# zhengjingsen/LidarDetection

Measured on AMD Instinct MI355X. Metric: frames/sec (fwd+NMS) PointPillar-KITTI, higher is better.
Workload: dtype f32; 1 GPU; PointPillar-KITTI bs=16 per GPU, fp32, eval BN folded: HIP voxelize + PFN; dense 2D backbone = first layer from the pillars (sparse implicit GEMM), stride-1 3x3 layers as Winograd F(4x4,3x3) on the fp32 MFMA, strided deblocks as one fused MFMA GEMM (all this repo's HIP), the two stride-2 3x3 layers MIOpen, stride-1 deblock + 1x1 heads hipBLASLt; exact HIP top-k + decode + batched rotated NMS; clou; replicas=1

## Files before the change

include/lidar_hip.h:

```cpp
#ifndef LIDAR_HIP_H
#define LIDAR_HIP_H

#include <stddef.h>
#include <stdint.h>

#ifdef __cplusplus
extern "C" {
#endif

#define LIDAR_OK 0
#define LIDAR_ERR_ARG (-1)
#define LIDAR_ERR_LAUNCH (-2)
#define LIDAR_ERR_WORKSPACE (-3)
#define LIDAR_ERR_UNSUPPORTED (-4)

size_t lidar_voxelize_workspace_bytes(int batch, int n_max, int max_voxels);
int lidar_voxelize_workspace_init(void *ws, size_t ws_bytes, int batch, int n_max, int max_voxels, void *stream);
int lidar_voxelize(const float *points, const int *point_offsets, int batch, int n_max, int num_features,
                   const float *range6, const float *voxel_size3, const int *grid3, int max_points,
                   int max_voxels, int compact, int algo, float *voxels, int *coords, int *num_points,
                   int *voxel_offsets, void *ws, size_t ws_bytes, void *stream);
int lidar_voxelize_hostoff(const float *points, const int *point_offsets, const int *host_offsets, int batch, int n_max,
                           int num_features, const float *range6, const float *voxel_size3, const int *grid3, int max_points,
                           int max_voxels, int compact, int algo, float *voxels, int *coords, int *num_points,
// ... 155 lines not shown
                               const float *weight, const float *bias, float *out_features, void *stream);
int lidar_spconv_implicit_gemm_fused(const float *in_features, const int *nbr, int n_out, int K, int Cin, int Cout,
                                     const float *weight, const float *bias, const float *residual, int relu,
                                     float *out_features, void *stream);
int lidar_spconv_row_masks(const int *nbr, int n_out, int K, int *masks, void *stream);
size_t lidar_spconv_mask_group_workspace_bytes(int n_out);
int lidar_spconv_mask_group_init(void *ws, size_t ws_bytes, void *stream);
int lidar_spconv_mask_group(const int *nbr, int n_out, int K, int *masks, int *order, void *ws, size_t ws_bytes, void *stream);
int lidar_spconv_sorted_gemm_supported(int K, int Cin, int Cout);
int lidar_spconv_implicit_gemm_sorted(const float *in_features, const int *nbr, const int *row_mask, const int *order,
                                      int n_out, int K, int Cin, int Cout, const float *weight, const float *bias,
                                      const float *residual, int relu, float *out_features, void *stream);
size_t lidar_spconv_packed_floats(int K, int Cin, int Cout);
int lidar_spconv_pack_weights(const float *weight, int K, int Cin, int Cout, float *packed, void *stream);
int lidar_spconv_implicit_gemm_sorted_packed(const float *in_features, const int *nbr, const int *row_mask, const int *order,
                                             int n_out, int K, int Cin, int Cout, const float *packed, const float *bias,
                                             const float *residual, int relu, float *out_features, void *stream);
int lidar_spconv_wgrad(const float *in_features, const float *grad_out, const int *nbr, int n_out, int K, int Cin, int Cout,
                       float *grad_weight, void *stream);
int lidar_spconv_wgrad_mfma_supported(int K, int Cin, int Cout);
size_t lidar_spconv_wgrad_workspace_bytes(int n_out, int K, int Cin, int Cout);
int lidar_spconv_wgrad_mfma(const float *in_features, const float *grad_out, const int *nbr, const int *order, int n_out, int K,
                            int Cin, int Cout, float *grad_weight, void *ws, size_t ws_bytes, void *stream);
size_t lidar_sparse_to_dense_workspace_bytes(int batch, int D, int H, int W);
int lidar_sparse_to_dense(const float *features, const int *indices, int n, int channels, int batch, int D, int H, int W,
                          float *out, void *ws, size_t ws_bytes, void *stream);

int lidar_bias_act_nhwc(const float *in, const float *bias, long long n_pix, int C, int relu, float *out, int out_C,
                        int out_off, void *stream);
int lidar_bias_act_upsample_nhwc(const float *in, const float *bias, int batch, int h, int w, int s, int C, int relu,
                                 float *out, int out_C, int out_off, void *stream);
int lidar_dense_gemm_bias_act(const float *A, long long M, int K, const float *W, int N, const float *bias, int relu,
                              float *D, int ldd, void *ws, size_t ws_bytes, void *stream);
int lidar_dense_gemm_export_choices(int *out7, int cap);
int lidar_dense_gemm_import_choices(const int *in7, int n);

size_t lidar_wino_packed_floats(int Cin, int Cout);
int lidar_wino_supported(int Cin, int Cout);
int lidar_wino_pack_weights(const float *w, int Cin, int Cout, float *packed, void *stream);
int lidar_wino_conv3x3_nhwc(const float *in, int B, int H, int W, int Cin, const float *packed, const float *bias, int relu, int Cout,
                            float *out, int out_C, int out_off, void *stream);
int lidar_wino_conv3x3_grouped_nhwc(const float *in, int B, int H, int W, int in_C, int group_cin, int n_groups, const float *packed,
                                    const float *bias, int relu, float *out, int out_C, int out_off, void *stream);
int lidar_wino_conv3x3_grouped_compact_nhwc(const float *in, int B, int H, int W, int in_C, int group_cin, int n_groups,
                                            const float *packed, const float *bias, int relu, const int *grp_cout, const int *grp_ooff,
                                            float *out, int out_C, int out_off, void *stream);

size_t lidar_wino43_packed_floats(int Cin, int Cout);
int lidar_wino43_supported(int Cin, int Cout);
int lidar_wino43_pack_weights(const float *w, int Cin, int Cout, float *packed, void *stream);
int lidar_wino43_conv3x3_nhwc(const float *in, int B, int H, int W, int Cin, int in_C, const float *packed, const float *bias, int relu,
                              int Cout, float *out, int out_C, int out_off, void *stream);

int lidar_wino43_wgrad_supported(int Cin, int Cout);
size_t lidar_wino43_wgrad_workspace_bytes(int B, int H, int W, int Cin, int Cout);
int lidar_wino43_wgrad_nhwc(const float *x, int x_ld, const float *g, int g_ld, int B, int H, int W, int Cin, int Cout, float *dw,
                            void *ws, size_t ws_bytes, void *stream);

size_t lidar_deconv_packed_floats(int K, int N);
int lidar_deconv_supported(int K, int s, int C_up);
int lidar_deconv_pack_weights(const float *W, int K, int N, float *packed, void *stream);
int lidar_deconv_gemm_nhwc(const float *in, int B, int h, int w, int K, const float *packed, const float *bias, int relu, int s, int C_up,
                           float *out, int out_C, int out_off, void *stream);

#define LIDAR_DECONV_TRAIN_MIN_K 16
#define LIDAR_DECONV_TRAIN_MIN_CUP 32
#define LIDAR_DECONV_TRAIN_MAX_C 512
int lidar_deconv_train_supported(int K, int s, int C_up);
size_t lidar_deconv_wgrad_workspace_bytes(int B, int h, int w, int K, int s, int C_up);
int lidar_deconv_dgrad_nhwc(const float *g, int g_ld, const float *W, int B, int h, int w, int K, int s, int C_up, float *dx, int dx_ld,
                            void *stream);
int lidar_deconv_wgrad_nhwc(const float *x, int x_ld, const float *g, int g_ld, int B, int h, int w, int K, int s, int C_up, float *dw,
                            void *ws, size_t ws_bytes, void *stream);

int lidar_anchor_scores(const float *head, long long n_loc, int row_stride, int cls_off, int anchors_per_loc, int num_class,
                        float score_thresh, float *scores, unsigned char *labels, void *stream);
int lidar_decode_topk(const float *head, int batch, long long locs_per_frame, int row_stride, int box_off, int dir_off,
                      int anchors_per_loc, int num_dir_bins, const long long *top_idx, int k, const float *anchors,
                      float dir_offset, float dir_limit_offset, float period, float *boxes, void *stream);
size_t lidar_topk_workspace_bytes(int batch, long long n);
int lidar_topk_workspace_init(void *ws, size_t ws_bytes, int batch, long long n, void *stream);
int lidar_anchor_scores_hist(const float *head, int batch, long long locs_per_frame, int row_stride, int cls_off, int anchors_per_loc,
                             int num_class, float score_thresh, float *scores, unsigned char *labels, void *ws, size_t ws_bytes,
                             void *stream);
int lidar_topk_desc(const float *scores, int batch, long long n, int k, float valid_min, float score_max, int hist_ready,
                    float *top_scores, long long *top_idx, int *counts, void *ws, size_t ws_bytes, void *stream);
int lidar_post_nms_gather(const float *boxes, const float *top_scores, const long long *top_idx, const unsigned char *labels,
                          const long long *keep, const int *num_keep, int batch, int k, long long n, int keep_stride, int post,
                          float *out_boxes, float *out_scores, long long *out_labels, int *out_num, void *stream);

size_t lidar_anchor_assign_workspace_bytes(int batch, int max_gt, int num_classes);
int lidar_anchor_assign(const float *const *anchors, const long long *counts, const long long *per_loc, const long long *out_off,
                        const float *matched, const float *unmatched, const int *remap, int num_classes, int anchor_dim,
                        long long a_total, const signed char *class_of_id, const float *gt, const float *gt_enlarged, int batch,
                        int max_gt, int gt_cols, int code_size, int sincos, int norm_by_num_examples, int *labels, float *targets,
                        float *weights, void *ws, size_t ws_bytes, void *stream);

size_t lidar_anchor_loss_workspace_bytes(int batch, const long long *counts, int num_heads);
int lidar_anchor_loss_forward(const float *const *cls, const float *const *box, const float *const *dir, const long long *counts,
                              const int *cols, const int *col_off, int num_heads, const int *labels, const float *targets,
                              const float *anchors, int anchor_dim, int batch, long long n_total, int num_class, int code_size,
                              int num_dir_bins, const float *code_weights, const float *weights, int flags, float *losses, void *ws,
                              size_t ws_bytes, void *stream);
int lidar_anchor_loss_backward(const float *const *cls, const float *const *box, const float *const *dir, const long long *counts,
                               const int *cols, const int *col_off, int num_heads, const int *labels, const float *targets,
                               const float *anchors, int anchor_dim, int batch, long long n_total, int num_class, int code_size,
// ... 17 lines not shown
```

lidardetection_amd/_lib.py:

```python
import ctypes as C
import os

_HERE = os.path.dirname(os.path.abspath(__file__))
SO_PATH = os.environ.get("LIDAR_HIP_SO") or os.path.join(_HERE, "csrc", "liblidar_hip.so")

vp, i32, f32, sz = C.c_void_p, C.c_int, C.c_float, C.c_size_t

SIGNATURES = {
    "lidar_voxelize_workspace_bytes": (sz, [i32, i32, i32]),
    "lidar_voxelize_workspace_init": (i32, [vp, sz, i32, i32, i32, vp]),
    "lidar_voxelize": (i32, [vp, vp, i32, i32, i32, vp, vp, vp, i32, i32, i32, i32, vp, vp, vp, vp, vp, sz, vp]),
    "lidar_voxelize_hostoff": (i32, [vp, vp, vp, i32, i32, i32, vp, vp, vp, i32, i32, i32, i32, vp, vp, vp, vp, vp, sz, vp]),
    "lidar_voxelize_error_flag": (i32, [vp, sz, i32, i32, i32]),
    "lidar_timer_create": (vp, []),
    "lidar_timer_destroy": (None, [vp]),
    "lidar_voxelize_time_next": (None, [vp]),
    "lidar_timer_elapsed_ms": (C.c_float, [vp]),
    "lidar_timer_parts_ms": (i32, [vp, vp]),
    "lidar_voxelize_set_error_mirror": (i32, [vp, sz, i32, i32, i32, vp, vp]),
    "lidar_pillar_vfe": (i32, [vp, vp, vp, i32, vp, i32, i32, vp, vp, vp, i32, vp, vp, i32, i32, i32, vp, vp]),
    "lidar_mean_vfe": (i32, [vp, vp, i32, i32, i32, i32, vp, vp]),
    "lidar_pillar_scatter_workspace_bytes": (sz, [i32, i32, i32]),
    "lidar_pillar_scatter": (i32, [vp, vp, i32, i32, vp, i32, i32, i32, i32, i32, vp, vp, sz, vp]),
    "lidar_pillar_scatter_update": (i32, [vp, vp, i32, i32, vp, i32, i32, i32, i32, vp, vp, vp, vp]),
# ... 35 lines not shown
    "lidar_gather_points_grad_batch": (i32, [i32, i32, i32, i32, vp, vp, vp, vp]),
    "lidar_three_nn_batch": (i32, [i32, i32, i32, vp, vp, vp, vp, vp]),
    "lidar_three_interpolate_batch": (i32, [i32, i32, i32, i32, vp, vp, vp, vp, vp]),
    "lidar_three_interpolate_grad_batch": (i32, [i32, i32, i32, i32, vp, vp, vp, vp, vp]),
    "lidar_roiaware_pool3d_forward": (i32, [i32, i32, i32, i32, i32, i32, i32, vp, vp, vp, vp, vp, vp, i32, vp]),
    "lidar_roiaware_pool3d_backward": (i32, [i32, i32, i32, i32, i32, i32, vp, vp, vp, vp, i32, vp]),
    "lidar_points_in_boxes": (i32, [i32, i32, i32, vp, vp, vp, vp]),
    "lidar_roipoint_pool3d_forward": (i32, [i32, i32, i32, i32, i32, vp, vp, vp, vp, vp, vp]),
    "lidar_spconv_hash_capacity": (sz, [i32]),
    "lidar_spconv_build_hash": (i32, [vp, i32, i32, i32, i32, vp, sz, vp]),
    "lidar_spconv_subm_table": (i32, [vp, i32, i32, i32, i32, i32, i32, i32, vp, sz, vp, vp]),
    "lidar_spconv_conv_table_workspace_bytes": (sz, [i32, i32, i32, i32, i32, i32, i32]),
    "lidar_spconv_conv_outputs": (i32, [vp, i32, i32, i32, i32, i32, i32, i32, i32, i32, i32, i32, i32, i32, i32, vp, i32, vp, vp, sz, vp]),
    "lidar_spconv_conv_tables": (i32, [i32, i32, i32, i32, i32, i32, i32, i32, vp, vp, vp, sz, vp]),
    "lidar_spconv_grid_init": (i32, [vp, sz, vp]),
    "lidar_spconv_grid_rows": (i32, [vp, i32, vp, i32, i32, i32, i32, vp, i32, vp]),
    "lidar_spconv_grid_table": (i32, [vp, i32, i32, i32, i32, i32, i32, i32, i32, i32, i32, i32, i32, i32, i32, vp, i32, vp, vp]),
    "lidar_spconv_grid_table_t": (i32, [vp, i32, i32, i32, i32, i32, i32, i32, i32, i32, i32, i32, i32, i32, i32, vp, i32, vp, vp]),
    "lidar_spconv_grid_pad_rows": (i32, [vp, vp, i32, vp]),
    "lidar_spconv_transpose_table": (i32, [vp, i32, i32, i32, vp, vp]),
    "lidar_spconv_grid_outputs_workspace_bytes": (sz, [i32, i32]),
    "lidar_spconv_grid_outputs": (i32, [vp, i32, i32, i32, i32, i32, i32, i32, i32, i32, i32, i32, i32, i32, i32, vp, vp, vp, vp, sz, vp]),
    "lidar_spconv_implicit_gemm": (i32, [vp, vp, i32, i32, i32, i32, vp, vp, vp, vp]),
    "lidar_spconv_implicit_gemm_fused": (i32, [vp, vp, i32, i32, i32, i32, vp, vp, vp, i32, vp, vp]),
    "lidar_spconv_row_masks": (i32, [vp, i32, i32, vp, vp]),
    "lidar_spconv_mask_group_workspace_bytes": (sz, [i32]),
    "lidar_spconv_mask_group_init": (i32, [vp, sz, vp]),
    "lidar_spconv_mask_group": (i32, [vp, i32, i32, vp, vp, vp, sz, vp]),
    "lidar_spconv_sorted_gemm_supported": (i32, [i32, i32, i32]),
    "lidar_spconv_implicit_gemm_sorted": (i32, [vp, vp, vp, vp, i32, i32, i32, i32, vp, vp, vp, i32, vp, vp]),
    "lidar_spconv_packed_floats": (sz, [i32, i32, i32]),
    "lidar_spconv_pack_weights": (i32, [vp, i32, i32, i32, vp, vp]),
    "lidar_spconv_implicit_gemm_sorted_packed": (i32, [vp, vp, vp, vp, i32, i32, i32, i32, vp, vp, vp, i32, vp, vp]),
    "lidar_spconv_wgrad": (i32, [vp, vp, vp, i32, i32, i32, i32, vp, vp]),
    "lidar_spconv_wgrad_mfma_supported": (i32, [i32, i32, i32]),
    "lidar_spconv_wgrad_workspace_bytes": (sz, [i32, i32, i32, i32]),
    "lidar_spconv_wgrad_mfma": (i32, [vp, vp, vp, vp, i32, i32, i32, i32, vp, vp, sz, vp]),
    "lidar_sparse_to_dense_workspace_bytes": (sz, [i32, i32, i32, i32]),
    "lidar_sparse_to_dense": (i32, [vp, vp, i32, i32, i32, i32, i32, i32, vp, vp, sz, vp]),
    "lidar_sparse_to_bev_nhwc": (i32, [vp, vp, i32, i32, i32, i32, i32, i32, vp, vp, sz, vp]),
    "lidar_bias_act_nhwc": (i32, [vp, vp, C.c_longlong, i32, i32, vp, i32, i32, vp]),
    "lidar_bias_act_upsample_nhwc": (i32, [vp, vp, i32, i32, i32, i32, i32, i32, vp, i32, i32, vp]),
    "lidar_dense_gemm_bias_act": (i32, [vp, C.c_longlong, i32, vp, i32, vp, i32, vp, i32, vp, sz, vp]),
    "lidar_dense_gemm_export_choices": (i32, [vp, i32]),
    "lidar_dense_gemm_import_choices": (i32, [vp, i32]),
    "lidar_wino_packed_floats": (sz, [i32, i32]),
    "lidar_wino_supported": (i32, [i32, i32]),
    "lidar_wino_pack_weights": (i32, [vp, i32, i32, vp, vp]),
    "lidar_wino_conv3x3_nhwc": (i32, [vp, i32, i32, i32, i32, vp, vp, i32, i32, vp, i32, i32, vp]),
    "lidar_wino43_packed_floats": (sz, [i32, i32]),
    "lidar_wino43_supported": (i32, [i32, i32]),
    "lidar_wino43_pack_weights": (i32, [vp, i32, i32, vp, vp]),
    "lidar_wino43_conv3x3_nhwc": (i32, [vp, i32, i32, i32, i32, i32, vp, vp, i32, i32, vp, i32, i32, vp]),
    "lidar_wino43_wgrad_supported": (i32, [i32, i32]),
    "lidar_wino43_wgrad_workspace_bytes": (sz, [i32, i32, i32, i32, i32]),
    "lidar_wino43_wgrad_nhwc": (i32, [vp, i32, vp, i32, i32, i32, i32, i32, i32, vp, vp, sz, vp]),
    "lidar_wino_conv3x3_grouped_nhwc": (i32, [vp, i32, i32, i32, i32, i32, i32, vp, vp, i32, vp, i32, i32, vp]),
    "lidar_wino_conv3x3_grouped_compact_nhwc": (i32, [vp, i32, i32, i32, i32, i32, i32, vp, vp, i32, vp, vp, vp, i32, i32, vp]),
    "lidar_deconv_packed_floats": (sz, [i32, i32]),
    "lidar_deconv_supported": (i32, [i32, i32, i32]),
    "lidar_deconv_pack_weights": (i32, [vp, i32, i32, vp, vp]),
    "lidar_deconv_gemm_nhwc": (i32, [vp, i32, i32, i32, i32, vp, vp, i32, i32, i32, vp, i32, i32, vp]),
    "lidar_deconv_train_supported": (i32, [i32, i32, i32]),
    "lidar_deconv_wgrad_workspace_bytes": (sz, [i32, i32, i32, i32, i32, i32]),
    "lidar_deconv_dgrad_nhwc": (i32, [vp, i32, vp, i32, i32, i32, i32, i32, i32, vp, i32, vp]),
    "lidar_deconv_wgrad_nhwc": (i32, [vp, i32, vp, i32, i32, i32, i32, i32, i32, i32, vp, vp, sz, vp]),
    "lidar_anchor_scores": (i32, [vp, C.c_longlong, i32, i32, i32, i32, f32, vp, vp, vp]),
    "lidar_decode_topk": (i32, [vp, i32, C.c_longlong, i32, i32, i32, i32, i32, vp, i32, vp, f32, f32, f32, vp, vp]),
    "lidar_topk_workspace_bytes": (sz, [i32, C.c_longlong]),
    "lidar_topk_workspace_init": (i32, [vp, sz, i32, C.c_longlong, vp]),
    "lidar_anchor_scores_hist": (i32, [vp, i32, C.c_longlong, i32, i32, i32, i32, f32, vp, vp, vp, sz, vp]),
    "lidar_topk_desc": (i32, [vp, i32, C.c_longlong, i32, f32, f32, i32, vp, vp, vp, vp, sz, vp]),
    "lidar_post_nms_gather": (i32, [vp, vp, vp, vp, vp, vp, i32, i32, C.c_longlong, i32, i32, vp, vp, vp, vp, vp]),
    "lidar_anchor_assign_workspace_bytes": (sz, [i32, i32, i32]),
    "lidar_anchor_assign": (i32, [vp, vp, vp, vp, vp, vp, vp, i32, i32, C.c_longlong, vp, vp, vp, i32, i32, i32, i32, i32, i32, vp,
                                  vp, vp, vp, sz, vp]),
    "lidar_anchor_loss_workspace_bytes": (sz, [i32, vp, i32]),
    "lidar_anchor_loss_forward": (i32, [vp, vp, vp, vp, vp, vp, i32, vp, vp, vp, i32, i32, C.c_longlong, i32, i32, i32, vp, vp, i32,
                                        vp, vp, sz, vp]),
    "lidar_anchor_loss_backward": (i32, [vp, vp, vp, vp, vp, vp, i32, vp, vp, vp, i32, i32, C.c_longlong, i32, i32, i32, vp, vp, i32,
                                         vp, vp, vp, vp, vp, sz, vp]),
    "lidar_rotate_iou_eval": (i32, [vp, i32, vp, i32, i32, vp, vp]),
    "lidar_boxes_iou_bev_cpu": (i32, [vp, i32, vp, i32, vp]),
    "lidar_points_in_boxes_cpu": (i32, [vp, i32, vp, i32, vp]),
    "lidar_voxelize_cpu_scratch_bytes": (sz, [i32]),
    "lidar_voxelize_cpu": (i32, [vp, i32, i32, vp, vp, vp, i32, i32, vp, vp, vp, vp, sz]),
}

_lib = None


class LidarHipError(RuntimeError):
    pass


def lib():
    global _lib
    if _lib is None:
        if not os.path.exists(SO_PATH):
            raise LidarHipError(
                f"{SO_PATH} is missing: build it with `python -c 'import __graft_entry__ as g; g.build()'` "
                "(hipcc --offload-arch=gfx950). There is no CPU fallback.")
        _lib = C.CDLL(SO_PATH)
        for name, (res, args) in SIGNATURES.items():
            fn = getattr(_lib, name)
            fn.restype = res
# ... 88 lines not shown
```

lidardetection_amd/bev_backbone.py:

```python
import ctypes as C
import os
from typing import NamedTuple, Optional

import torch
import torch.nn as nn
import torch.nn.functional as F

from . import _lib, wino, workspace


def bias_act_(x, bias, relu=True, out=None, out_offset=0):
    _lib.require_cuda(bias)
    if not (x.is_cuda and x.dim() == 4 and x.is_contiguous(memory_format=torch.channels_last)):
        raise _lib.LidarHipError("bias_act_: expected a channels-last CUDA tensor")
    B, C, H, W = x.shape
    out, out_offset = (x, 0) if out is None else _lib.nhwc_out("bias_act_", B, (H, W), C, x.device, out, out_offset)
    _lib.check(_lib.lib().lidar_bias_act_nhwc(_lib.ptr(x), _lib.ptr(bias), B * H * W, C, int(bool(relu)), _lib.ptr(out),
                                              out.shape[1], int(out_offset), _lib.stream()), "lidar_bias_act_nhwc")
    return out


_LT_GEMM = [os.environ.get("LIDAR_BEV_LT_GEMM", "1") != "0"]
_SPLIT_MIN = [int(os.environ.get("LIDAR_BEV_SPLIT_MIN", "8"))]
_SPLIT = [int(os.environ.get("LIDAR_BEV_SPLIT", "2"))]
_WINO = [os.environ.get("LIDAR_BEV_WINO", "1") != "0"]
_DECONV = [os.environ.get("LIDAR_BEV_DECONV", "1") != "0"]
_SPARSE_FIRST = [os.environ.get("LIDAR_BEV_SPARSE_FIRST", "1") != "0"]


def _lt_gemm(a_ptr, M, K, w_kn, bias, relu, d_ptr, ldd, device):
    ws = workspace.get("dense_gemm", 32 << 20, device)
    st = _lib.lib().lidar_dense_gemm_bias_act(a_ptr, M, K, _lib.ptr(w_kn), w_kn.shape[1], _lib.ptr(bias), int(bool(relu)), d_ptr, ldd,
                                              _lib.ptr(ws), ws.numel(), _lib.stream())
    if st == -4:
        return False
    _lib.check(st, "lidar_dense_gemm_bias_act")
    return True


def _side_streams(device, n):
    from .spconv import conv as _sc, modules as _sm
    dev = torch.device(device)
    out = []
    for pool in (_sc._SIDE_STREAMS, _sm._RULEBOOK_STREAMS)[:n]:
        st = pool.get(dev)
        if st is None:
            st = pool[dev] = torch.cuda.Stream(dev, priority=-1)
        out.append(st)
    return out


def gemm_bias_act_into_(x, w_kn, bias, out, out_offset, relu=True):
    _lib.require_cuda(w_kn, bias)
    _lib.require_nhwc(x, "gemm_bias_act_into_")
    B, K, h, w = x.shape
    N = w_kn.shape[1]
    if w_kn.shape[0] != K or bias.numel() != N:
        raise _lib.LidarHipError("gemm_bias_act_into_: shapes do not match")
    out, out_offset = _lib.nhwc_out("gemm_bias_act_into_", B, (h, w), N, x.device, out, out_offset)
    return _lt_gemm(_lib.ptr(x), B * h * w, K, w_kn, bias, relu, C.c_void_p(out.data_ptr() + 4 * out_offset), out.shape[1], x.device)


def rows_gemm(a2d, w_kn, bias=None, out=None):
    if _LT_GEMM[0] and a2d.is_cuda and a2d.dtype == torch.float32 and a2d.is_contiguous() and w_kn.is_contiguous():
        if out is None:
            out = torch.empty((a2d.shape[0], w_kn.shape[1]), dtype=torch.float32, device=a2d.device)
        elif not out.is_contiguous() or out.shape != (a2d.shape[0], w_kn.shape[1]):
            raise _lib.LidarHipError("rows_gemm: out must be a contiguous (M, N) tensor")
        if _lt_gemm(_lib.ptr(a2d), a2d.shape[0], a2d.shape[1], w_kn, bias, False, _lib.ptr(out), w_kn.shape[1], a2d.device):
            return out
        _LT_GEMM[0] = False
    if out is None:
        return torch.mm(a2d, w_kn) if bias is None else torch.addmm(bias, a2d, w_kn)
    return torch.mm(a2d, w_kn, out=out) if bias is None else torch.addmm(bias, a2d, w_kn, out=out)


def deconv_supported(K, s, c_up):
    return bool(_lib.lib().lidar_deconv_supported(int(K), int(s), int(c_up)))


def deconv_pack(w_kn):
    _lib.require_cuda(w_kn)
    K, N = w_kn.shape
    L = _lib.lib()
    n = L.lidar_deconv_packed_floats(K, N)
    if n == 0:
        raise _lib.LidarHipError(f"deconv_pack: unsupported shape ({K}, {N})")
    packed = torch.empty(n, dtype=torch.float32, device=w_kn.device)
    _lib.check(L.lidar_deconv_pack_weights(_lib.ptr(w_kn.contiguous()), K, N, _lib.ptr(packed), _lib.stream()), "lidar_deconv_pack_weights")
    return packed


_DECONV_MAX_BYTES = [2 ** 31 - 1]


def deconv_fits(B, K, h, w, s, out_c):
    return B * h * w * K * 4 < _DECONV_MAX_BYTES[0] and B * h * w * s * s * out_c * 4 < _DECONV_MAX_BYTES[0]


def deconv_gemm_into_(x, packed, bias, s, out, out_offset=0, relu=True):
    _lib.require_cuda(packed, bias)
    _lib.require_nhwc(x, "deconv_gemm_into_")
    B, K, h, w = x.shape
    c_up = bias.numel()
    if packed.numel() != K * s * s * c_up:
        raise _lib.LidarHipError("deconv_gemm_into_: packed weights do not match (K, s, C_up)")
    out, out_offset = _lib.nhwc_out("deconv_gemm_into_", B, (s * h, s * w), c_up, x.device, out, out_offset)
    _lib.check(_lib.lib().lidar_deconv_gemm_nhwc(_lib.ptr(x), B, h, w, K, _lib.ptr(packed), _lib.ptr(bias), int(bool(relu)), int(s), c_up,
                                                 _lib.ptr(out), out.shape[1], int(out_offset), _lib.stream()), "lidar_deconv_gemm_nhwc")
    return out


def bias_act_upsample_(y2d, bias, batch, h, w, s, out, out_offset=0, relu=True):
    _lib.require_cuda(y2d, bias)
    C = bias.numel()
    if y2d.shape != (batch * h * w, s * s * C):
        raise _lib.LidarHipError("bias_act_upsample_: GEMM output shape does not match (batch*h*w, s*s*C)")
    out, out_offset = _lib.nhwc_out("bias_act_upsample_", batch, (h * s, w * s), C, y2d.device, out, out_offset)
    _lib.check(_lib.lib().lidar_bias_act_upsample_nhwc(_lib.ptr(y2d), _lib.ptr(bias), batch, h, w, s, C, int(bool(relu)),
                                                       _lib.ptr(out), out.shape[1], int(out_offset), _lib.stream()),
               "lidar_bias_act_upsample_nhwc")
    return out


def collect_params(*modules):
    out = []
    for m in modules:
        out += list(m.parameters()) + list(m.buffers())
    return out


def params_key(tensors):
    return tuple((t.data_ptr(), t._version) for t in tensors)


def _fold(weight, bn, out_dim, conv_bias=None):
    scale = bn.weight.detach() / torch.sqrt(bn.running_var + bn.eps)
    shift = bn.bias.detach() - bn.running_mean * scale
    if conv_bias is not None:
        shift = shift + conv_bias.detach() * scale
    shape = [1] * weight.dim()
    shape[out_dim] = -1
    return (weight.detach() * scale.view(shape)), shift.contiguous()


class BlockLayer(NamedTuple):
    zpad: Optional[nn.ZeroPad2d]
    conv: nn.Conv2d
    bn: nn.BatchNorm2d
    act: Optional[nn.ReLU]
    pad: Optional[tuple]
    zero_pad: Optional[tuple]

    @property
    def plain3x3(self):
        c = self.conv
        return (self.pad == (1, 1) and self.zero_pad is None and tuple(c.kernel_size) == (3, 3) and tuple(c.stride) == (1, 1)
                and tuple(c.dilation) == (1, 1) and c.groups == 1)


def block_layer(zpad, conv, bn, act=None):
    pad, zero_pad = None, None if zpad is None else tuple(int(v) for v in zpad.padding)
    if conv.padding_mode == "zeros" and not isinstance(conv.padding, str):
        pad = tuple(int(v) for v in conv.padding)
        if zero_pad is not None and zero_pad[0] == zero_pad[1] >= 0 and zero_pad[2] == zero_pad[3] >= 0:
            pad, zero_pad = (pad[0] + zero_pad[2], pad[1] + zero_pad[0]), None
    return BlockLayer(zpad, conv, bn, act, pad, zero_pad)


def parse_block(blk):
    mods, out, i = list(blk), [], 0
    while i < len(mods):
        zpad = None
        if isinstance(mods[i], nn.ZeroPad2d):
            zpad, i = mods[i], i + 1
        if i + 3 > len(mods):
            return None
        conv, bn, act = mods[i:i + 3]
        if not (isinstance(conv, nn.Conv2d) and isinstance(bn, nn.BatchNorm2d) and isinstance(act, nn.ReLU)):
            return None
        out.append(block_layer(zpad, conv, bn, act))
        i += 3
    return out


class FoldedConv(NamedTuple):
    weight: torch.Tensor
    shift: torch.Tensor
    stride: tuple
    pad: tuple
    dilation: tuple
    groups: int
    zero_pad: Optional[tuple]
    wino: Optional[list]


class FoldedDeblock(NamedTuple):
    kind: str
    weight: torch.Tensor
    packed: Optional[torch.Tensor]
    shift: torch.Tensor
    stride: int
    args: tuple


def _cl(t):
    return t if t.is_contiguous(memory_format=torch.channels_last) else t.contiguous(memory_format=torch.channels_last)


class FoldedBEVBackbone:

    def __init__(self, blocks, deblocks, heads):
        self.sources = collect_params(blocks, deblocks, *heads)
        self.source_key = params_key(self.sources)
        self.stages = []
        for blk, de in zip(blocks, deblocks):
            layers = parse_block(blk)
            assert layers is not None, "FoldedBEVBackbone: blocks must be [ZeroPad2d] Conv2d BatchNorm2d ReLU groups"
            convs = []
            for l in layers:
                assert l.pad is not None, "FoldedBEVBackbone: explicit zero padding only"
                w, b = _fold(l.conv.weight, l.bn, 0, l.conv.bias)
                packed = None
                if _WINO[0] and w.is_cuda and l.plain3x3 and wino.supported(w.shape[1], w.shape[0]):
                    packed = wino.pack_auto(w)
                convs.append(FoldedConv(w.contiguous(memory_format=torch.channels_last), b, tuple(l.conv.stride), l.pad,
                                        tuple(l.conv.dilation), l.conv.groups, l.zero_pad, packed))
            up, bn = de[0], de[1]
            assert tuple(up.dilation) == (1, 1) and up.groups == 1 and up.padding_mode == "zeros", \
                "FoldedBEVBackbone: deblocks with dilation, groups or non-zero padding modes are not supported"
            if isinstance(up, nn.ConvTranspose2d):
                w, b = _fold(up.weight, bn, 1, up.bias)
                s = up.stride[0]
                if tuple(up.kernel_size) == tuple(up.stride) and s == up.stride[1] and \
                        tuple(up.padding) == (0, 0) and tuple(up.output_padding) == (0, 0):
                    w_kn = w.permute(0, 2, 3, 1).reshape(w.shape[0], -1).contiguous()
                    upc = FoldedDeblock("gemm", w_kn, None, b, s, ())
                    if _DECONV[0] and w.is_cuda and s > 1 and deconv_supported(w_kn.shape[0], s, b.numel()):
                        upc = upc._replace(kind="deconv_mfma", packed=deconv_pack(w_kn))
                else:
                    upc = FoldedDeblock("deconv", w.contiguous(memory_format=torch.channels_last), None, b, 0,
                                        (up.stride, up.padding, up.output_padding))
            else:
                w, b = _fold(up.weight, bn, 0, up.bias)
                upc = FoldedDeblock("conv", w.contiguous(memory_format=torch.channels_last), None, b, 0, (up.stride, up.padding))
            self.stages.append((convs, upc))
        self.up_channels = [up.shift.numel() for _, up in self.stages]
        for h in heads:
            assert tuple(h.kernel_size) == (1, 1) and tuple(h.stride) == (1, 1)
        self.head_split = [h.weight.shape[0] for h in heads]
        if heads:
            self.head_wt = torch.cat([h.weight.detach().flatten(1) for h in heads], 0).t().contiguous()
            self.head_b = torch.cat([h.bias.detach() if h.bias is not None else h.weight.new_zeros(h.weight.shape[0])
                                     for h in heads], 0).contiguous()
        self._cats = {}
        self._streams = None
        self._first_sparse = None
        c0 = self.stages[0][0][0]
        w0, b0, st0, pad0 = c0.weight, c0.shift, c0.stride, c0.pad
        k0 = w0.shape[2]
        if (w0.is_cuda and w0.shape[2] == w0.shape[3] and st0[0] == st0[1] and pad0[0] == pad0[1] and k0 * k0 <= 31
                and c0.dilation == (1, 1) and c0.groups == 1 and c0.zero_pad is None):
            from .spconv import ops as _sops
            if _sops.sorted_gemm_supported(k0 * k0, w0.shape[1], w0.shape[0]):
                self._first_sparse = (w0.permute(2, 3, 1, 0).reshape(k0 * k0, w0.shape[1], w0.shape[0]).contiguous(), b0, k0, int(st0[0]), int(pad0[0]))

    def first_layer_from_pillars(self, pm):
        from . import pillar_ops
        from .spconv import ops as _sops
        w9, b0, k0, st0, pad0 = self._first_sparse
        nbr, OH, OW = pillar_ops.pillar_conv_table(pm.coords, pm.B, pm.nx, pm.ny, k0, st0, pad0, pm.num_voxels_dev)
        order = _sops.mask_order(nbr)
        out = _sops.indice_conv_fused(pm.features, nbr, w9, b0, None, True, order)
        return out.view(pm.B, OH, OW, w9.shape[2]).permute(0, 3, 1, 2)

    def sparse_first_ok(self):
        return self._first_sparse is not None and _SPARSE_FIRST[0]

    def features(self, canvas, slot=0, first_done=False):
        x, cat, off = canvas, None, 0
        for si, (convs, up) in enumerate(self.stages):
            for ci, cv in enumerate(convs):
                if first_done and si == 0 and ci == 0:
                    continue
                if cv.wino is not None and _WINO[0] and x.is_contiguous(memory_format=torch.channels_last):
                    x = wino.conv3x3_auto(x, cv.wino, cv.weight.shape[0], cv.shift, True)
                    continue
                if cv.zero_pad is not None:
                    x = F.pad(x, cv.zero_pad)
                x = _cl(F.conv2d(x, cv.weight, None, cv.stride, cv.pad, cv.dilation, cv.groups))
                bias_act_(x, cv.shift)
            B, _, h, w = x.shape
            y = None
            if up.kind in ("deconv", "conv"):
                y = _cl((F.conv_transpose2d if up.kind == "deconv" else F.conv2d)(x, up.weight, None, *up.args))
            oh, ow = (h * up.stride, w * up.stride) if y is None else y.shape[2:]
            if cat is None:
                shape = (B, sum(self.up_channels), oh, ow)
                cat = self._cats.get(slot)
                if cat is None or cat.shape != shape or cat.device != x.device:
                    cat = self._cats[slot] = torch.empty(shape, dtype=torch.float32, device=x.device,
                                                         memory_format=torch.channels_last)
            if y is not None:
                bias_act_(y, up.shift, out=cat, out_offset=off)
            else:
                self._deblock_gemm(x, up, cat, off)
            off += up.shift.numel()
        return cat

    def _deblock_gemm(self, x, up, cat, off):
        B, K, h, w = x.shape
        if up.kind == "deconv_mfma" and deconv_fits(B, K, h, w, up.stride, cat.shape[1]):
            return deconv_gemm_into_(x, up.packed, up.shift, up.stride, cat, off)
        if up.kind == "gemm" and up.stride == 1 and _LT_GEMM[0]:
            if gemm_bias_act_into_(x, up.weight, up.shift, cat, off):
                return cat
            _LT_GEMM[0] = False
        y = rows_gemm(x.permute(0, 2, 3, 1).reshape(B * h * w, -1), up.weight)
        return bias_act_upsample_(y, up.shift, B, h, w, up.stride, cat, off)

    def stale(self):
        return params_key(self.sources) != self.source_key

    def merged(self, canvas):
        first_done = False
        if not torch.is_tensor(canvas):
            if self.sparse_first_ok():
                canvas, first_done = self.first_layer_from_pillars(canvas), True
            else:
                canvas = canvas.dense()
        B = canvas.shape[0]
        if 1 < _SPLIT[0] <= 2 and canvas.is_cuda and B % _SPLIT[0] == 0 and B // _SPLIT[0] >= _SPLIT_MIN[0]:
            return self._merged_split(canvas, _SPLIT[0], first_done)
        cat = self.features(canvas, first_done=first_done)
        B, C, H, W = cat.shape
        out = rows_gemm(cat.permute(0, 2, 3, 1).reshape(B * H * W, C), self.head_wt, self.head_b)
        return out.view(B, H, W, -1)

    def _merged_split(self, canvas, n, first_done=False):
        dev = canvas.device
# ... 22 lines not shown
```

lidardetection_amd/csrc/build.py:

```python
import glob
import os
import subprocess
import sys

HERE = os.path.dirname(os.path.abspath(__file__))
SO = os.path.join(HERE, "liblidar_hip.so")
HIPCC = os.environ.get("HIPCC", "/opt/rocm/bin/hipcc")
FLAGS = ["--offload-arch=gfx950", "-O3", "-fPIC", "-std=c++17", "-ffp-contract=off", "-fvisibility=hidden",
         "-Wall", "-Wno-unused-function"]
EXTRA_FLAGS = {"wino43_conv.hip": ["-mllvm", "-pragma-unroll-threshold=4000000", "-Wno-inline-asm"]}


def sources():
    return sorted(glob.glob(os.path.join(HERE, "*.hip")))


def build(force=False, verbose=False):
    srcs = sources()
    deps = srcs + glob.glob(os.path.join(HERE, "*.h")) + [os.path.abspath(__file__)]
    if not force and os.path.exists(SO) and all(os.path.getmtime(SO) >= os.path.getmtime(d) for d in deps):
        return SO
    objs = []
    procs = []
    for s in srcs:
        o = s[:-4] + ".o"
        if (not force and os.path.exists(o)
                and all(os.path.getmtime(o) >= os.path.getmtime(d) for d in [s] + deps[len(srcs):])):
            objs.append(o)
            continue
        cmd = [HIPCC, *FLAGS, *EXTRA_FLAGS.get(os.path.basename(s), []), "-c", s, "-o", o]
        if verbose:
            print(" ".join(cmd))
        procs.append((s, subprocess.Popen(cmd)))
        objs.append(o)
    for s, p in procs:
        if p.wait() != 0:
            raise RuntimeError(f"hipcc failed on {s}")
    cmd = [HIPCC, "--offload-arch=gfx950", "-shared", "-fPIC", "-o", SO, *objs]
    if verbose:
        print(" ".join(cmd))
    subprocess.check_call(cmd)
    return SO


VARIANTS = {
    "vxl_nowait": ("voxelize.hip", ["-DVXL_WAIT_TICKS=0"]),
}
AB_VARIANTS = {
    "w43_aux0": ("wino43_conv.hip", ["-DW43_STORE_AUX=0"]),
    "vxl_fill_nt": ("voxelize.hip", ["-DVXL_FILL_NT=1"]),
    "vxl_share12": ("voxelize.hip", ["-DVXL_FILL_SHARE16=12"]), "vxl_share10": ("voxelize.hip", ["-DVXL_FILL_SHARE16=10"]),
    "vxl_share8": ("voxelize.hip", ["-DVXL_FILL_SHARE16=8"]),
    "dc_nowait": ("deconv_gemm.hip", ["-DDC_PROBE=1"]),
    "sc_p1": ("sparse_conv.hip", ["-DSC_PROBE=1"]), "sc_p2": ("sparse_conv.hip", ["-DSC_PROBE=2"]), "sc_p4": ("sparse_conv.hip", ["-DSC_PROBE=4"]),
    "sc_p7": ("sparse_conv.hip", ["-DSC_PROBE=7"]),
}


def variant_path(name):
    return os.path.join(HERE, f"liblidar_hip_{name}.so")


def build_variants(force=False, verbose=False, names=None):
# ... 25 lines not shown
```

Baseline: 3248 frames/s.

## Add HIP MFMA direct kernel for stride-2 3x3 conv replacing MIOpen

Adds a HIP direct-convolution kernel for stride-2 3x3 layers. It uses fp32 MFMA, double-buffered LDS input tiles loaded by buffer-to-LDS DMA, and fused bias+ReLU with an NHWC output offset. By default it replaces the MIOpen call only for the stride-2 layer with Cin<=64, aiming to cut MIOpen overhead and layout handling. The wider layer stays on MIOpen unless LIDAR_BEV_S2=all is set. This adds inline-asm complexity and risks being slower than MIOpen's tuned kernels.

```diff
diff --git a/include/lidar_hip.h b/include/lidar_hip.h
--- a/include/lidar_hip.h
+++ b/include/lidar_hip.h
@@ -231,6 +231,12 @@
 int lidar_wino43_conv3x3_nhwc(const float *in, int B, int H, int W, int Cin, int in_C, const float *packed, const float *bias, int relu,
                               int Cout, float *out, int out_C, int out_off, void *stream);
 
+size_t lidar_conv3x3s2_packed_floats(int Cin, int Cout);
+int lidar_conv3x3s2_supported(int Cin, int Cout);
+int lidar_conv3x3s2_pack_weights(const float *w, int Cin, int Cout, float *packed, void *stream);
+int lidar_conv3x3s2_nhwc(const float *in, int B, int H, int W, int Cin, int in_C, const float *packed, const float *bias, int relu,
+                         int Cout, float *out, int out_C, int out_off, void *stream);
+
 int lidar_wino43_wgrad_supported(int Cin, int Cout);
 size_t lidar_wino43_wgrad_workspace_bytes(int B, int H, int W, int Cin, int Cout);
 int lidar_wino43_wgrad_nhwc(const float *x, int x_ld, const float *g, int g_ld, int B, int H, int W, int Cin, int Cout, float *dw,
diff --git a/lidardetection_amd/_lib.py b/lidardetection_amd/_lib.py
--- a/lidardetection_amd/_lib.py
+++ b/lidardetection_amd/_lib.py
@@ -111,6 +111,10 @@
     "lidar_wino43_supported": (i32, [i32, i32]),
     "lidar_wino43_pack_weights": (i32, [vp, i32, i32, vp, vp]),
     "lidar_wino43_conv3x3_nhwc": (i32, [vp, i32, i32, i32, i32, i32, vp, vp, i32, i32, vp, i32, i32, vp]),
+    "lidar_conv3x3s2_packed_floats": (sz, [i32, i32]),
+    "lidar_conv3x3s2_supported": (i32, [i32, i32]),
+    "lidar_conv3x3s2_pack_weights": (i32, [vp, i32, i32, vp, vp]),
+    "lidar_conv3x3s2_nhwc": (i32, [vp, i32, i32, i32, i32, i32, vp, vp, i32, i32, vp, i32, i32, vp]),
     "lidar_wino43_wgrad_supported": (i32, [i32, i32]),
     "lidar_wino43_wgrad_workspace_bytes": (sz, [i32, i32, i32, i32, i32]),
     "lidar_wino43_wgrad_nhwc": (i32, [vp, i32, vp, i32, i32, i32, i32, i32, i32, vp, vp, sz, vp]),
diff --git a/lidardetection_amd/bev_backbone.py b/lidardetection_amd/bev_backbone.py
--- a/lidardetection_amd/bev_backbone.py
+++ b/lidardetection_amd/bev_backbone.py
@@ -25,6 +25,8 @@
 _SPLIT = [int(os.environ.get("LIDAR_BEV_SPLIT", "2"))]
 _WINO = [os.environ.get("LIDAR_BEV_WINO", "1") != "0"]
 _DECONV = [os.environ.get("LIDAR_BEV_DECONV", "1") != "0"]
+_S2 = [os.environ.get("LIDAR_BEV_S2", "1") != "0"]
+_S2_MAX_CIN = [256 if os.environ.get("LIDAR_BEV_S2", "1") == "all" else 64]
 _SPARSE_FIRST = [os.environ.get("LIDAR_BEV_SPARSE_FIRST", "1") != "0"]
 
 
@@ -111,6 +113,44 @@
     return out
 
 
+def conv_s2_supported(cin, cout):
+    return bool(_lib.lib().lidar_conv3x3s2_supported(int(cin), int(cout)))
+
+
+def conv_s2_pack(w):
+    _lib.require_cuda(w.contiguous())
+    cout, cin = w.shape[:2]
+    L = _lib.lib()
+    n = L.lidar_conv3x3s2_packed_floats(cin, cout)
+    if n == 0 or tuple(w.shape[2:]) != (3, 3):
+        raise _lib.LidarHipError(f"conv_s2_pack: unsupported weight {tuple(w.shape)}")
+    packed = torch.empty(n, dtype=torch.float32, device=w.device)
+    _lib.check(L.lidar_conv3x3s2_pack_weights(_lib.ptr(w.contiguous()), cin, cout, _lib.ptr(packed), _lib.stream()), "lidar_conv3x3s2_pack_weights")
+    return packed
+
+
+_S2_MAX_BYTES = [2 ** 31 - 1]
+
+
+def conv_s2_fits(B, in_c, H, W, out_c):
+    oh, ow = (H - 1) // 2 + 1, (W - 1) // 2 + 1
+    return B * H * W * in_c * 4 < _S2_MAX_BYTES[0] and B * oh * ow * out_c * 4 < _S2_MAX_BYTES[0]
+
+
+def conv_s2_(x, packed, bias, relu=True, out=None, out_offset=0):
+    _lib.require_cuda(packed, bias)
+    in_c = _lib.nhwc_ld(x, "conv_s2_")
+    B, cin, H, W = x.shape
+    cout = bias.numel()
+    if packed.numel() != 9 * cin * cout:
+        raise _lib.LidarHipError("conv_s2_: packed weights do not match (Cin, Cout)")
+    oh, ow = (H - 1) // 2 + 1, (W - 1) // 2 + 1
+    out, out_offset = _lib.nhwc_out("conv_s2_", B, (oh, ow), cout, x.device, out, out_offset)
+    _lib.check(_lib.lib().lidar_conv3x3s2_nhwc(_lib.ptr(x), B, H, W, cin, in_c, _lib.ptr(packed), _lib.ptr(bias), int(bool(relu)), cout,
+                                               _lib.ptr(out), out.shape[1], int(out_offset), _lib.stream()), "lidar_conv3x3s2_nhwc")
+    return out
+
+
 def bias_act_upsample_(y2d, bias, batch, h, w, s, out, out_offset=0, relu=True):
     _lib.require_cuda(y2d, bias)
     C = bias.numel()
@@ -151,6 +191,12 @@
     act: Optional[nn.ReLU]
     pad: Optional[tuple]
     zero_pad: Optional[tuple]
+
+    @property
+    def s2_3x3(self):
+        c = self.conv
+        return (self.pad == (1, 1) and self.zero_pad is None and tuple(c.kernel_size) == (3, 3) and tuple(c.stride) == (2, 2)
+                and tuple(c.dilation) == (1, 1) and c.groups == 1)
 
     @property
     def plain3x3(self):
@@ -193,6 +239,7 @@
     groups: int
     zero_pad: Optional[tuple]
     wino: Optional[list]
+    s2: Optional[torch.Tensor] = None
 
 
 class FoldedDeblock(NamedTuple):
@@ -224,8 +271,11 @@
                 packed = None
                 if _WINO[0] and w.is_cuda and l.plain3x3 and wino.supported(w.shape[1], w.shape[0]):
                     packed = wino.pack_auto(w)
+                s2 = None
+                if _S2[0] and w.is_cuda and l.s2_3x3 and conv_s2_supported(w.shape[1], w.shape[0]):
+                    s2 = conv_s2_pack(w)
                 convs.append(FoldedConv(w.contiguous(memory_format=torch.channels_last), b, tuple(l.conv.stride), l.pad,
-                                        tuple(l.conv.dilation), l.conv.groups, l.zero_pad, packed))
+                                        tuple(l.conv.dilation), l.conv.groups, l.zero_pad, packed, s2))
             up, bn = de[0], de[1]
             assert tuple(up.dilation) == (1, 1) and up.groups == 1 and up.padding_mode == "zeros", \
                 "FoldedBEVBackbone: deblocks with dilation, groups or non-zero padding modes are not supported"
@@ -286,6 +336,10 @@
                 if cv.wino is not None and _WINO[0] and x.is_contiguous(memory_format=torch.channels_last):
                     x = wino.conv3x3_auto(x, cv.wino, cv.weight.shape[0], cv.shift, True)
                     continue
+                if (cv.s2 is not None and _S2[0] and x.shape[1] <= _S2_MAX_CIN[0] and x.is_contiguous(memory_format=torch.channels_last)
+                        and conv_s2_fits(x.shape[0], x.shape[1], x.shape[2], x.shape[3], cv.weight.shape[0])):
+                    x = conv_s2_(x, cv.s2, cv.shift, True)
+                    continue
                 if cv.zero_pad is not None:
                     x = F.pad(x, cv.zero_pad)
                 x = _cl(F.conv2d(x, cv.weight, None, cv.stride, cv.pad, cv.dilation, cv.groups))
diff --git a/lidardetection_amd/csrc/build.py b/lidardetection_amd/csrc/build.py
--- a/lidardetection_amd/csrc/build.py
+++ b/lidardetection_amd/csrc/build.py
@@ -8,7 +8,8 @@
 HIPCC = os.environ.get("HIPCC", "/opt/rocm/bin/hipcc")
 FLAGS = ["--offload-arch=gfx950", "-O3", "-fPIC", "-std=c++17", "-ffp-contract=off", "-fvisibility=hidden",
          "-Wall", "-Wno-unused-function"]
-EXTRA_FLAGS = {"wino43_conv.hip": ["-mllvm", "-pragma-unroll-threshold=4000000", "-Wno-inline-asm"]}
+EXTRA_FLAGS = {"wino43_conv.hip": ["-mllvm", "-pragma-unroll-threshold=4000000", "-Wno-inline-asm"],
+               "conv3x3s2.hip": ["-Wno-inline-asm"]}
 
 
 def sources():
diff --git a/lidardetection_amd/csrc/conv3x3s2.hip b/lidardetection_amd/csrc/conv3x3s2.hip
--- /dev/null
+++ b/lidardetection_amd/csrc/conv3x3s2.hip
@@ -0,0 +1,216 @@
+#include "common.h"
+
+typedef float f32x4 __attribute__((ext_vector_type(4)));
+typedef int i32x4 __attribute__((ext_vector_type(4)));
+
+#define CS_OOB 0x80000000u
+#define CS_NF 3
+#define CS_MIN_CIN 32
+#define CS_MAX_C 256
+
+static constexpr int cs_npix(int FW) { return (2 * (2 * CS_NF * (16 / FW)) + 1) * (2 * FW + 1); }
+static constexpr int cs_plane(int FW) { return (cs_npix(FW) + 14) / 16 * 16 + 1; }
+static constexpr int cs_qw(int FW) { return (4 * cs_plane(FW) + 255) / 256; }
+
+__global__ __launch_bounds__(256) void cs_pack_kernel(const float *__restrict__ w, int Cin, int Cout, float *__restrict__ P) {
+    const long long idx = (long long)blockIdx.x * 256 + threadIdx.x;
+    if (idx >= 9ll * Cin * Cout) return;
+    const int j = (int)(idx & 3), lane = (int)((idx >> 2) & 63), nt = Cout >> 4;
+    int rest = (int)(idx >> 8);
+    const int T = rest % nt;
+    rest /= nt;
+    const int tap = rest % 9, c = rest / 9;
+    const int co = 16 * T + (lane & 15), ch = 16 * c + 4 * (lane >> 4) + j;
+    P[idx] = w[((size_t)co * Cin + ch) * 9 + tap];
+}
+
+struct CsArgs {
+    const float *in;
+    const float *pk;
+    const float *bias;
+    float *out;
+    int B, H, W, Cin, in_C, Cout, OH, OW, out_C, out_off, relu;
+    int tiles_x, tiles_y, ncg;
+    unsigned in_bytes;
+};
+
+template <int FW>
+__global__ __launch_bounds__(256, 2) void cs_conv_kernel(const CsArgs a) {
+    constexpr int FR = 16 / FW, NF = CS_NF, TH = 2 * NF * FR;
+    constexpr int RW = 2 * FW + 1, NPIX = cs_npix(FW), PLANE = cs_plane(FW), QW = cs_qw(FW), STAGE = QW * 256;
+    __shared__ float4 s_img[2 * STAGE];
+
+    const int t = threadIdx.x, l = t & 63, wv = __builtin_amdgcn_readfirstlane(t >> 6);
+    const int wm = wv >> 1, wn = wv & 1;
+    const int i = l & 15, kq = l >> 4;
+    const int H = a.H, W = a.W;
+
+    int blk = (int)blockIdx.x;
+    const int cg = blk % a.ncg;
+    blk /= a.ncg;
+    const int tx = blk % a.tiles_x;
+    blk /= a.tiles_x;
+    const int ty = blk % a.tiles_y, b = blk / a.tiles_y;
+    const int oy0 = ty * TH, ox0 = tx * FW;
+
+    unsigned doff[QW];
+#pragma unroll
+    for (int k = 0; k < QW; ++k) {
+        const int s = (wv + 4 * k) * 64 + l;
+        const int pl = s / PLANE, p = s - pl * PLANE;
+        const int ry = p / RW, rx = p - ry * RW;
+        const int gy = 2 * oy0 - 1 + ry, gx = 2 * ox0 - 1 + rx;
+        const bool ok = pl < 4 && p < NPIX && gy >= 0 && gy < H && gx >= 0 && gx < W;
+        doff[k] = ok ? ((unsigned)((b * H + gy) * W + gx) * (unsigned)a.in_C + 4u * (unsigned)pl) * 4u : CS_OOB;
+    }
+    i32x4 rsrc;
+    {
+        const unsigned long long base = (unsigned long long)a.in;
+        rsrc[0] = (int)(unsigned)base;
+        rsrc[1] = (int)((unsigned)(base >> 32) & 0xffffu);
+        rsrc[2] = (int)a.in_bytes;
+        rsrc[3] = 0x00020000;
+    }
+    const unsigned img_lds = (unsigned)(size_t)((__attribute__((address_space(3))) char *)s_img);
+    auto dma = [&](int buf) {
+#pragma unroll
+        for (int k = 0; k < QW; ++k) {
+            const unsigned dst = img_lds + (unsigned)((buf * STAGE + (wv + 4 * k) * 64) * 16);
+            asm volatile("s_mov_b32 m0, %2\n\ts_nop 0\n\tbuffer_load_dwordx4 %0, %1, 0 offen lds" : : "v"(doff[k]), "s"(rsrc), "s"(dst) : "memory", "m0");
+            doff[k] += 64u;
+        }
+    };
+
+    const int T0 = cg * 8 + wn * 4;
+    const bool active = 16 * T0 < a.Cout;
+    const int nt = a.Cout >> 4;
+    const __amdgpu_buffer_rsrc_t frsrc = __builtin_amdgcn_make_buffer_rsrc(const_cast<float *>(a.pk), (short)0, (int)(9u * (unsigned)a.Cin * (unsigned)a.Cout * 4u), 0x00020000);
+    const int l16 = l * 16;
+    auto ldw = [&](int f4_index) { return __builtin_bit_cast(f32x4, __builtin_amdgcn_raw_buffer_load_b128(frsrc, l16, f4_index * 16, 0)); };
+    int xb[NF];
+#pragma unroll
+    for (int rr = 0; rr < NF; ++rr) {
+        const int f = wm * NF + rr;
+        xb[rr] = kq * PLANE + 2 * (f * FR + i / FW) * RW + 2 * (i % FW);
+    }
+
+    f32x4 acc[4][NF];
+#pragma unroll
+    for (int tt = 0; tt < 4; ++tt)
+#pragma unroll
+        for (int rr = 0; rr < NF; ++rr) acc[tt][rr] = (f32x4){0.f, 0.f, 0.f, 0.f};
+
+    const int NC = a.Cin >> 4;
+    dma(0);
+    for (int c = 0; c < NC; ++c) {
+        asm volatile("s_waitcnt vmcnt(0) lgkmcnt(0)\n\ts_barrier" ::: "memory");
+        const float4 *img = s_img + (c & 1) * STAGE;
+        f32x4 wc[4], xc[NF], wx[4], xx[NF];
+        if (active) {
+            const int wbase = (c * 9 * nt + T0) * 64;
+#pragma unroll
+            for (int tt = 0; tt < 4; ++tt) wc[tt] = ldw(wbase + tt * 64);
+#pragma unroll
+            for (int rr = 0; rr < NF; ++rr) xc[rr] = __builtin_bit_cast(f32x4, img[xb[rr]]);
+        }
+        __builtin_amdgcn_sched_barrier(0);
+        if (c + 1 < NC) dma((c + 1) & 1);
+        __builtin_amdgcn_sched_barrier(0);
+        if (active) {
+            const int wbase = (c * 9 * nt + T0) * 64;
+#pragma unroll
+            for (int tap = 0; tap < 9; ++tap) {
+                if (tap < 8) {
+                    const int ky = (tap + 1) / 3, kx = (tap + 1) % 3;
+#pragma unroll
+                    for (int tt = 0; tt < 4; ++tt) wx[tt] = ldw(wbase + ((tap + 1) * nt + tt) * 64);
+#pragma unroll
+                    for (int rr = 0; rr < NF; ++rr) xx[rr] = __builtin_bit_cast(f32x4, img[xb[rr] + ky * RW + kx]);
+                }
+                __builtin_amdgcn_sched_barrier(0);
+#pragma unroll
+                for (int j = 0; j < 4; ++j)
+#pragma unroll
+                    for (int tt = 0; tt < 4; ++tt)
+#pragma unroll
+                        for (int rr = 0; rr < NF; ++rr)
+                            acc[tt][rr] = __builtin_amdgcn_mfma_f32_16x16x4f32(wc[tt][j], xc[rr][j], acc[tt][rr], 0, 0, 0);
+                __builtin_amdgcn_sched_barrier(0);
+                if (tap < 8) {
+#pragma unroll
+                    for (int tt = 0; tt < 4; ++tt) wc[tt] = wx[tt];
+#pragma unroll
+                    for (int rr = 0; rr < NF; ++rr) xc[rr] = xx[rr];
+                }
+            }
+        }
+    }
+
+    if (!active) return;
+    const bool relu = a.relu != 0;
+    const int cw = cg * 128 + wn * 64 + 4 * kq;
+    f32x4 sh[4];
+#pragma unroll
+    for (int tt = 0; tt < 4; ++tt)
+#pragma unroll
+        for (int r = 0; r < 4; ++r) sh[tt][r] = a.bias ? a.bias[cw + 16 * tt + r] : 0.f;
+#pragma unroll
+    for (int rr = 0; rr < NF; ++rr) {
+        const int f = wm * NF + rr;
+        const int oy = oy0 + f * FR + i / FW, ox = ox0 + i % FW;
+        if (oy >= a.OH || ox >= a.OW) continue;
+        float *o = a.out + ((size_t)(b * a.OH + oy) * a.OW + ox) * a.out_C + a.out_off + cw;
+#pragma unroll
+        for (int tt = 0; tt < 4; ++tt) {
+            f32x4 v = acc[tt][rr] + sh[tt];
+            if (relu) {
+#pragma unroll
+                for (int r = 0; r < 4; ++r) v[r] = fmaxf(v[r], 0.f);
+            }
+            *reinterpret_cast<f32x4 *>(o + 16 * tt) = v;
+        }
+    }
+}
+
+LIDAR_EXPORT int lidar_conv3x3s2_supported(int Cin, int Cout) {
+    return Cin >= CS_MIN_CIN && Cin <= CS_MAX_C && (Cin & 15) == 0 && Cout >= 64 && Cout <= CS_MAX_C && (Cout & 63) == 0;
+}
+
+LIDAR_EXPORT size_t lidar_conv3x3s2_packed_floats(int Cin, int Cout) {
+    return lidar_conv3x3s2_supported(Cin, Cout) ? (size_t)9 * Cin * Cout : 0;
+}
+
+LIDAR_EXPORT int lidar_conv3x3s2_pack_weights(const float *w, int Cin, int Cout, float *packed, void *stream) {
+    if (!w || !packed) return LIDAR_ERR_ARG;
+    if (!lidar_conv3x3s2_supported(Cin, Cout)) return LIDAR_ERR_UNSUPPORTED;
+    hipLaunchKernelGGL(cs_pack_kernel, dim3(divup(9ll * Cin * Cout, 256)), dim3(256), 0, (hipStream_t)stream, w, Cin, Cout, packed);
+    return lidar_check_launch("lidar_conv3x3s2_pack_weights");
+}
+
+LIDAR_EXPORT int lidar_conv3x3s2_nhwc(const float *in, int B, int H, int W, int Cin, int in_C, const float *packed, const float *bias, int relu,
+                                      int Cout, float *out, int out_C, int out_off, void *stream) {
+    if (!in || !packed || !out || B <= 0 || H <= 0 || W <= 0 || Cin <= 0 || Cout <= 0 || in_C < Cin || out_off < 0 ||
+        (long long)out_off + Cout > out_C)
+        return LIDAR_ERR_ARG;
+    if ((reinterpret_cast<uintptr_t>(in) & 15) || (reinterpret_cast<uintptr_t>(packed) & 15) || (reinterpret_cast<uintptr_t>(out) & 15) ||
+        (in_C & 3) || (out_C & 3) || (out_off & 3))
+        return LIDAR_ERR_ARG;
+    if (!lidar_conv3x3s2_supported(Cin, Cout)) return LIDAR_ERR_UNSUPPORTED;
+    const int OH = (H - 1) / 2 + 1, OW = (W - 1) / 2 + 1;
+    if ((long long)B * H * W * in_C * 4 >= 0x7fffffffll || (long long)B * OH * OW * out_C * 4 >= 0x7fffffffll)
+        return LIDAR_ERR_UNSUPPORTED;
+    CsArgs a;
+    a.in = in; a.pk = packed; a.bias = bias; a.out = out;
+    a.B = B; a.H = H; a.W = W; a.Cin = Cin; a.in_C = in_C; a.Cout = Cout; a.OH = OH; a.OW = OW; a.out_C = out_C; a.out_off = out_off; a.relu = relu;
+    a.in_bytes = (unsigned)((long long)B * H * W * in_C * 4);
+    a.ncg = divup(Cout, 128);
+    const long long t16 = (long long)divup(OH, 2 * CS_NF) * divup(OW, 16), t8 = (long long)divup(OH, 4 * CS_NF) * divup(OW, 8);
+    const bool fw8 = t8 < t16;
+    a.tiles_y = fw8 ? divup(OH, 4 * CS_NF) : divup(OH, 2 * CS_NF);
+    a.tiles_x = fw8 ? divup(OW, 8) : divup(OW, 16);
+    const long long grid = (long long)B * a.tiles_y * a.tiles_x * a.ncg;
+    if (grid > 0x7fffffffll) return LIDAR_ERR_UNSUPPORTED;
+    if (fw8) hipLaunchKernelGGL(cs_conv_kernel<8>, dim3((unsigned)grid), dim3(256), 0, (hipStream_t)stream, a);
+    else hipLaunchKernelGGL(cs_conv_kernel<16>, dim3((unsigned)grid), dim3(256), 0, (hipStream_t)stream, a);
+    return lidar_check_launch("lidar_conv3x3s2_nhwc");
+}
```

After: 3267 frames/s, median of 6. No clear change (+0.6%).
